# harmony-one/harmony

Measured on AMD Instinct MI355X. Metric: BLS12-381 aggregate-verifies/sec (committee=4096), higher is better.
Workload: dtype u64; 1 GPU; config2: committee=4096 masked aggregate + pairing verify, batch=262144/step, masks Bernoulli(0.9) seed 42, 48B staking commit payloads; parallelism=dp1 (per-shard replicas, no collective)

## Files before the change

### harmony_amd/core.py

```python
import ctypes
import os

_DIR = os.path.dirname(os.path.abspath(__file__))
_SO = os.environ.get("HBLS_SO", os.path.join(_DIR, "libhbls.so"))

HBLS_OK = 1
HBLS_FALSE = 0
HBLS_ERR = -1
HBLS_ERR_NOGPU = -2
HBLS_ERR_BADINPUT = -3
HBLS_NOQUORUM = -4
NOQUORUM = HBLS_NOQUORUM
TWO_THIRDS_DEC = 666666666666666667


class HblsError(RuntimeError):
    pass


class NoGpuError(HblsError):
    pass


class BadInputError(HblsError, ValueError):
# ... 68 lines not shown
    lib.hbls_vote_key_sums.argtypes = [
        ctypes.c_void_p, ctypes.POINTER(ctypes.c_uint32),
        ctypes.POINTER(ctypes.c_uint32), ctypes.c_size_t, ctypes.c_char_p,
        ctypes.POINTER(ctypes.c_int32)]
    lib.hbls_batch_verify_votes_multi.argtypes = [
        ctypes.c_void_p, ctypes.POINTER(ctypes.c_uint32),
        ctypes.POINTER(ctypes.c_uint32), ctypes.c_char_p, ctypes.c_char_p,
        ctypes.c_size_t, ctypes.c_size_t, ctypes.POINTER(ctypes.c_int32)]
    lib.hbls_stream_process_multi.argtypes = [
        ctypes.c_void_p, ctypes.POINTER(ctypes.c_uint32),
        ctypes.POINTER(ctypes.c_uint32), ctypes.POINTER(ctypes.c_uint32),
        ctypes.c_char_p, ctypes.POINTER(ctypes.c_uint32), ctypes.c_int,
        ctypes.c_size_t, ctypes.POINTER(ctypes.c_int32)]
    lib.hbls_rlc_last_stats.argtypes = [ctypes.POINTER(ctypes.c_uint32)]
    lib.hbls_rlc_last_stats.restype = None
    lib.hbls_set_agg_verify_mode.argtypes = [ctypes.c_int]
    lib.hbls_set_aggrlc_threshold.argtypes = [ctypes.c_int]
    lib.hbls_set_aggrlc_threshold.restype = None
    lib.hbls_aggrlc_last_stats.argtypes = [ctypes.POINTER(ctypes.c_uint32)]
    lib.hbls_aggrlc_last_stats.restype = None
    lib.hbls_set_aggrlc_final.argtypes = [ctypes.c_int]
    lib.hbls_aggrlc_final_selftest.argtypes = [ctypes.c_int]
    lib.hbls_set_aggrlc_sigleg.argtypes = [ctypes.c_int]
    lib.hbls_aggrlc_probe.argtypes = [ctypes.c_int, ctypes.c_char_p, ctypes.c_size_t,
                                      ctypes.c_char_p]
    lib.hbls_last_host_ns.restype = ctypes.c_uint64
    lib.hbls_last_host_ns.argtypes = [ctypes.c_int]
    u64p, u32p, i32p = (ctypes.POINTER(t) for t in
                        (ctypes.c_uint64, ctypes.c_uint32, ctypes.c_int32))
    lib.hbls_committee_set_quorum.argtypes = [ctypes.c_void_p, u64p, ctypes.c_uint64]
    lib.hbls_mask_power.argtypes = [ctypes.c_void_p, ctypes.c_char_p, ctypes.c_size_t,
                                    u64p, u32p]
    lib.hbls_agg_verify_quorum.argtypes = lib.hbls_agg_verify.argtypes
    lib.hbls_batch_agg_verify_quorum.argtypes = lib.hbls_batch_agg_verify.argtypes
    lib.hbls_batch_seal_verify_quorum.argtypes = lib.hbls_batch_seal_verify.argtypes
    lib.hbls_stream_power.argtypes = [ctypes.c_void_p, u32p, ctypes.c_int,
                                      u64p, u32p, i32p]
    lib.hbls_last_stage_ns.argtypes = [ctypes.c_int]
    lib.hbls_copy_bench_ns.restype = ctypes.c_uint64
    lib.hbls_copy_bench_ns.argtypes = [ctypes.c_size_t]
    lib.hbls_fpmul_bench_waves.restype = ctypes.c_double
    lib.hbls_fpmul_bench_waves.argtypes = [ctypes.c_int, ctypes.c_int]
    lib.hbls_coop_selftest.restype = ctypes.c_int
    lib.hbls_fpmul_asm_check.restype = ctypes.c_longlong
    lib.hbls_arith_probe.argtypes = [ctypes.c_int, ctypes.c_char_p, ctypes.c_size_t,
                                     ctypes.c_char_p, i32p]
# ... 76 lines not shown

def aggrlc_chunk_size() -> int:
    return _lib.hbls_aggrlc_chunk_size()


def aggrlc_last_stats():
    out = (ctypes.c_uint32 * 3)()
    _lib.hbls_aggrlc_last_stats(out)
    return list(out)


def set_aggrlc_final(kernel: int):
    _check(_lib.hbls_set_aggrlc_final(kernel), "set_aggrlc_final")


def aggrlc_final_selftest(nchunks: int) -> int:
    return _check(_lib.hbls_aggrlc_final_selftest(nchunks), "aggrlc_final_selftest")


def set_aggrlc_sigleg(leg: int):
    _check(_lib.hbls_set_aggrlc_sigleg(leg), "set_aggrlc_sigleg")


AGGRLC_PROBE_OPS = {"g1_mul64w": (0, 3 * 48 + 8, 3 * 48),
                    "g2_mul64w": (1, 6 * 48 + 8, 6 * 48),
                    "miller1_fe": (2, 6 * 48, 12 * 48)}


def aggrlc_probe(name: str, data: bytes, n_items: int) -> bytes:
    op, in_b, out_b = AGGRLC_PROBE_OPS[name]
    if len(data) != n_items * in_b:
        raise ValueError("aggrlc_probe: operand size")
    out = ctypes.create_string_buffer(max(1, n_items * out_b))
    _check(_lib.hbls_aggrlc_probe(op, data, n_items, out), "aggrlc_probe")
    return out.raw[:n_items * out_b]


def last_host_ns(i: int) -> int:
    return _lib.hbls_last_host_ns(i)


def pk_from_sk(sk32: bytes) -> bytes:
    out = ctypes.create_string_buffer(48)
    _check(_lib.hbls_pk_from_sk(sk32, out), "pk_from_sk")
    return out.raw

# ... 489 lines not shown
```

### harmony_amd/csrc/hbls_aggrlc.inc

```

#define AGGRLC_CHUNK 64
#define AGGRLC_WINDOWS 8


DEV void aggrlc_recode64(uint64_t k, uint64_t &mag, uint32_t &neg, uint32_t &top) {
    uint32_t c = 0;
    mag = 0; neg = 0;
#pragma unroll
    for (int j = 0; j < 16; j++) {
        uint32_t v = ((uint32_t)(k >> (4 * j)) & 15u) + c;
        uint32_t nx = j < 15 ? ((uint32_t)(k >> (4 * j + 4)) & 15u) : 0u;
        c = (v > 8u || (v == 8u && nx >= 8u)) ? 1u : 0u;
        uint32_t m = c ? 16u - v : v;
        mag |= (uint64_t)m << (4 * j);
        neg |= (c && m) ? (1u << j) : 0u;
    }
    top = c;
}

DEVN void g1_mul64w(g1_t &r, const g1_t &p, uint64_t k) {
    g1_t tab[8];
    tab[0] = p;
    g1_dbl(tab[1], tab[0]);
    g1_add(tab[2], tab[1], tab[0]);
// ... 104 lines not shown
    g1aff_t pa, ca;
    { fp_t t, ti, zi, zi2, zi3;
      fp_mul(t, A.z, C.z);
      fp_inv(ti, t);
      fp_mul(zi, ti, C.z);
      fp_sqr(zi2, zi);
      fp_mul(zi3, zi2, zi);
      fp_mul(pa.x, A.x, zi2);
      fp_mul(pa.y, A.y, zi3);
      fp_mul(zi, ti, A.z);
      fp_sqr(zi2, zi);
      fp_mul(zi3, zi2, zi);
      fp_mul(ca.x, C.x, zi2);
      fp_mul(ca.y, C.y, zi3); }
    g2aff_t ha;
    g2_t hmc = hms[i];
    g2_to_affine(ha, hmc);
    miller_loop2(f, ha, pa, sigs[i], ca);
    F[i] = f;
    elig[i] = 1;
    results[i] = 1;
}

__global__ void k_aggrlc_sigscale(const g1_t *aggpubs, const g2aff_t *sigs,
                                  const int32_t *sig_flags, const int32_t *hm_ok,
                                  const uint64_t *scalars, g2_t *B, int32_t *elig,
                                  int32_t *results, int batch) {
    int i = blockIdx.x * blockDim.x + threadIdx.x;
    if (i >= batch) return;
    g2_t b;
    g2_set_inf(b);
    elig[i] = 0;
    if (!hm_ok[i] || sig_flags[i] == 0) {
        results[i] = HBLS_ERR_BADINPUT; B[i] = b; return;
    }
    bool sig_inf = sig_flags[i] == 2;
    bool pub_inf = g1_is_inf(aggpubs[i]);
    if (pub_inf || sig_inf) {
        results[i] = (pub_inf && sig_inf) ? 1 : 0;
        B[i] = b; return;
    }
    uint64_t r = scalars[i];
    if (r == 0) r = 1;
    g2_t s;
    g2_from_affine(s, sigs[i]);
    g2_mul64w(b, s, r);
    B[i] = b;
    elig[i] = 1;
    results[i] = 1;
}

__global__ void __launch_bounds__(AGGRLC_CHUNK) k_aggrlc_sigsum(
        const g2_t *B, int batch, int nchunks, g2aff_t *S, int32_t *sflag) {
    int c = blockIdx.x;
    if (c >= nchunks) return;
    __shared__ g2_t red[AGGRLC_CHUNK];
    size_t i = (size_t)c * AGGRLC_CHUNK + threadIdx.x;
    if (i < (size_t)batch) red[threadIdx.x] = B[i];
    else g2_set_inf(red[threadIdx.x]);
    __syncthreads();
    for (int s = AGGRLC_CHUNK / 2; s > 0; s >>= 1) {
        if (threadIdx.x < s) {
            g2_t t;
            g2_add(t, red[threadIdx.x], red[threadIdx.x + s]);
            red[threadIdx.x] = t;
        }
        __syncthreads();
    }
    if (threadIdx.x == 0) {
        g2_t sum = red[0];
        if (g2_is_inf(sum)) {
            sflag[c] = 0;
        } else {
            g2aff_t a;
            g2_to_affine(a, sum);
            S[c] = a;
            sflag[c] = 1;
        }
    }
}

__global__ void k_aggrlc_miller1(const g1_t *aggpubs, const g2_t *hms,
                                 const uint64_t *scalars, const g2aff_t *S,
                                 const int32_t *sflag, fp12_t *F, int32_t *elig,
                                 int32_t *results, int batch, int nchunks) {
    size_t i = (size_t)blockIdx.x * blockDim.x + threadIdx.x;
    if (i >= (size_t)batch + (size_t)nchunks) return;
    fp12_t f;
    g2aff_t Q;
    g1aff_t P;
    bool run = false;
    if (i < (size_t)batch) {
        if (elig[i] == 1) {
            uint64_t r = scalars[i];
            if (r == 0) r = 1;
            g1_t A;
            g1_mul64w(A, aggpubs[i], r);
            if (g1_is_inf(A)) {
                elig[i] = 2; results[i] = 0;
            } else {
                g1_to_affine(P, A);
                g2_t hmc = hms[i];
                g2_to_affine(Q, hmc);
                run = true;
            }
        }
    } else {
        size_t c = i - (size_t)batch;
        if (sflag[c]) {
            Q = S[c];
            fp_load(P.x, BLS_G1_X);
            fp_t gy;
            fp_load(gy, BLS_G1_Y);
            fp_neg(P.y, gy);
            run = true;
        }
    }
    if (run) miller_loop1_h(f, Q, P);
    else fp12_one(f);
    F[i] = f;
}

__global__ void __launch_bounds__(AGGRLC_CHUNK) k_aggrlc_chunk_prod(
        const fp12_t *F, const int32_t *elig, int batch, int nchunks,
        fp12_t *FC, int32_t *ccnt, int32_t *cforce, const fp12_t *FX) {
    int c = blockIdx.x;
    if (c >= nchunks) return;
    __shared__ fp12_t red[AGGRLC_CHUNK];
    size_t i = (size_t)c * AGGRLC_CHUNK + threadIdx.x;
    int e = i < (size_t)batch ? elig[i] : 0;
    if (e == 1) red[threadIdx.x] = F[i];
    else fp12_one(red[threadIdx.x]);
    int cnt = __syncthreads_count(e != 0);
    int force = __syncthreads_or(e == 2);
    for (int s = AGGRLC_CHUNK / 2; s > 0; s >>= 1) {
        if (threadIdx.x < s) {
            fp12_t t;
            fp12_mul(t, red[threadIdx.x], red[threadIdx.x + s]);
            red[threadIdx.x] = t;
        }
        __syncthreads();
    }
    if (threadIdx.x == 0) {
// ... 111 lines not shown
    return g_aggrlc_final;
}
extern "C" int hbls_set_aggrlc_final(int kernel) {
    if (kernel == -1) kernel = AGGRLC_FINAL_DEFAULT;
    if (kernel != 0 && kernel != 8 && kernel != 16) return HBLS_ERR_BADINPUT;
    g_aggrlc_final = kernel;
    return HBLS_OK;
}
#define AGGRLC_SIGLEG_MIN_BATCH 16384
static int g_aggrlc_sigleg = -2;
static int aggrlc_sigleg(size_t batch) {
    if (g_aggrlc_sigleg == -2) {
        const char *e = getenv("HBLS_AGGRLC_SIGLEG");
        int k = e ? atoi(e) : -1;
        g_aggrlc_sigleg = (k == 0 || k == 1) ? k : -1;
    }
    if (g_aggrlc_sigleg >= 0) return g_aggrlc_sigleg;
    return batch >= AGGRLC_SIGLEG_MIN_BATCH ? 1 : 0;
}
extern "C" int hbls_set_aggrlc_sigleg(int leg) {
    if (leg < -1 || leg > 1) return HBLS_ERR_BADINPUT;
    g_aggrlc_sigleg = leg;
    return HBLS_OK;
}

static void launch_aggrlc_final(int kernel, const fp12_t *d_FC, const int32_t *d_ccnt,
                                const int32_t *d_cforce, int32_t *d_verdict, int nc) {
    if (kernel == 16)
        hipLaunchKernelGGL(k_aggrlc_final_coop<16>, dim3((uint32_t)((nc + 15) / 16)),
                           dim3(16 * CV_LANES), 0, 0, d_FC, d_ccnt, d_cforce, d_verdict, nc);
    else if (kernel == 8)
        hipLaunchKernelGGL(k_aggrlc_final_coop<8>, dim3((uint32_t)((nc + 7) / 8)),
                           dim3(8 * CV_LANES), 0, 0, d_FC, d_ccnt, d_cforce, d_verdict, nc);
    else
        hipLaunchKernelGGL(k_aggrlc_final, dim3((uint32_t)((nc + 63) / 64)), dim3(64), 0, 0,
                           d_FC, d_ccnt, d_cforce, d_verdict, nc);
}

__global__ void k_aggrlc_final_fill(fp12_t *FC, int32_t *ccnt, int32_t *cforce, int nchunks) {
    int c = blockIdx.x * blockDim.x + threadIdx.x;
    if (c >= nchunks) return;
    int kind = c % 8;
    fp_t one;
    fp_one(one);
    fp_t co[12];
    for (int k = 0; k < 12; k++) {
// ... 65 lines not shown
                       dp2.as<g1aff_t>(), 64, dwj.as<g1_t>(), AGGRLC_WINDOWS);
    hipLaunchKernelGGL(k_wtab_to_affine, dim3((int)((m + 255) / 256)), dim3(256), 0, 0,
                       dwj.as<g1_t>(), d_gt, dwi.as<uint8_t>(), m);
    std::vector<uint8_t> winf(m);
    bool ok = hipDeviceSynchronize() == hipSuccess &&
              hipMemcpy(winf.data(), dwi.p, m, hipMemcpyDeviceToHost) == hipSuccess;
    for (size_t k = 0; ok && k < m; k++)
        if (winf[k]) ok = false;
    if (!ok) { hipFree(d_gt); return HBLS_ERR; }
    g_aggrlc_gtab = d_gt;
    return HBLS_OK;
}

static bool aggrlc_wanted(size_t batch) {
    int m = agg_verify_mode();
    if (m == 0 || !g_aggrlc_gtab) return false;
    if (batch > RLC_MAX_ITEMS || (long long)batch < (long long)g_aggrlc_threshold) return false;
    if (m == 1) return true;
    return (int)batch > coop_threshold() && rf_mode() == 0 && !use_batch_affine();
}

static int aggrlc_verify(const g1_t *d_agg, const g2_t *d_hm, const g2aff_t *d_saff,
                         const int32_t *d_sflags, const int32_t *d_hok,
                         int32_t *d_res, size_t batch) {
    size_t nc = (batch + AGGRLC_CHUNK - 1) / AGGRLC_CHUNK;
    const int leg = aggrlc_sigleg(batch);
    const size_t nx = leg ? nc : 0;
    std::vector<uint64_t> scalars(batch);
    if (!rlc_draw_scalars(scalars.data(), batch)) return AGGRLC_FALLBACK;
    FreeClock fclk;
    uint64_t t_alloc = host_now_ns();
    const size_t f_bytes = (batch + nx) * sizeof(fp12_t);
    const size_t b_bytes = leg ? batch * sizeof(g2_t) : 0;
    DevBuf dsc(batch * 8), dF(f_bytes + b_bytes + nx * sizeof(g2aff_t)), delig(batch * 4);
    DevBuf dFC(nc * sizeof(fp12_t)), dcs((3 * nc + nx) * 4);
    g_host_ns[0] += host_now_ns() - t_alloc;
    FreeClockArm farm(fclk);
    if (dsc.err || dF.err || delig.err || dFC.err || dcs.err) {
        (void)hipGetLastError();
        return AGGRLC_FALLBACK;
    }
    fp12_t *d_F = dF.as<fp12_t>();
    g2_t *d_B = (g2_t *)((uint8_t *)dF.p + f_bytes);
    g2aff_t *d_S = (g2aff_t *)((uint8_t *)dF.p + f_bytes + b_bytes);
    EventSet<1> up;
    if (up.err != hipSuccess) return HBLS_ERR;
    HIP_OK(upload_then_wait(dsc.p, scalars.data(), batch * 8, up[0]));
    int32_t *d_ccnt = dcs.as<int32_t>(), *d_cforce = d_ccnt + nc, *d_verdict = d_cforce + nc;
    int32_t *d_sf = d_verdict + nc;
    EventSet<5> ev;
    if (ev.err != hipSuccess) return HBLS_ERR;
    (void)hipEventRecord(ev[0], 0);
    if (leg) {
        hipLaunchKernelGGL(k_aggrlc_sigscale, dim3((uint32_t)((batch + 63) / 64)), dim3(64), 0, 0,
                           d_agg, d_saff, d_sflags, d_hok, dsc.as<uint64_t>(), d_B,
                           delig.as<int32_t>(), d_res, (int)batch);
        hipLaunchKernelGGL(k_aggrlc_sigsum, dim3((uint32_t)nc), dim3(AGGRLC_CHUNK), 0, 0,
                           d_B, (int)batch, (int)nc, d_S, d_sf);
    }
    (void)hipEventRecord(ev[1], 0);
    if (leg)
        hipLaunchKernelGGL(k_aggrlc_miller1, dim3((uint32_t)((batch + nc + 63) / 64)), dim3(64),
                           0, 0, d_agg, d_hm, dsc.as<uint64_t>(), d_S, d_sf, d_F,
                           delig.as<int32_t>(), d_res, (int)batch, (int)nc);
    else
        hipLaunchKernelGGL(k_aggrlc_miller, dim3((uint32_t)((batch + 63) / 64)), dim3(64), 0, 0,
                           d_agg, d_hm, d_saff, d_sflags, d_hok, dsc.as<uint64_t>(),
                           g_aggrlc_gtab, d_F, delig.as<int32_t>(), d_res, (int)batch);
    (void)hipEventRecord(ev[2], 0);
    hipLaunchKernelGGL(k_aggrlc_chunk_prod, dim3((uint32_t)nc), dim3(AGGRLC_CHUNK), 0, 0,
                       d_F, delig.as<int32_t>(), (int)batch, (int)nc,
                       dFC.as<fp12_t>(), d_ccnt, d_cforce,
                       leg ? d_F + batch : (const fp12_t *)nullptr);
    (void)hipEventRecord(ev[3], 0);
    launch_aggrlc_final(aggrlc_final_kernel(), dFC.as<fp12_t>(), d_ccnt, d_cforce,
                        d_verdict, (int)nc);
    (void)hipEventRecord(ev[4], 0);
    std::vector<int32_t> hc(3 * nc);
    hipError_t e = hipMemcpy(hc.data(), dcs.p, 3 * nc * 4, hipMemcpyDeviceToHost);
    if (e == hipSuccess) e = hipGetLastError();
    for (int i = 0; i < 4; i++) {
        float ms = 0;
        if (e == hipSuccess && (i || leg)) (void)hipEventElapsedTime(&ms, ev[i], ev[i + 1]);
        g_stage_ns[i ? 3 + i : 7] = (uint64_t)(ms * 1e6);
    }
    HIP_OK(e);

    std::vector<uint32_t> failed;
    for (size_t c = 0; c < nc; c++) {
        if (hc[c] <= 0) continue;
        g_aggrlc_stats[0]++;
        if (hc[2 * nc + c] == 1) continue;
        g_aggrlc_stats[1]++;
        failed.push_back((uint32_t)c);
    }
    if (failed.empty()) return HBLS_OK;

    std::vector<int32_t> helig(batch);
    HIP_OK(hipMemcpy(helig.data(), delig.p, batch * 4, hipMemcpyDeviceToHost));
    std::vector<uint32_t> sel;
    for (uint32_t c : failed)
        for (size_t i = (size_t)c * AGGRLC_CHUNK;
             i < batch && i < ((size_t)c + 1) * AGGRLC_CHUNK; i++)
            if (helig[i]) sel.push_back((uint32_t)i);
    size_t ns = sel.size();
    g_aggrlc_stats[2] = (uint32_t)ns;
    if (!ns) return HBLS_OK;
    DevBuf dsel(ns * 4);
    if (dsel.err) return HBLS_ERR;
    HIP_OK(hipMemcpy(dsel.p, sel.data(), ns * 4, hipMemcpyHostToDevice));
    hipLaunchKernelGGL(k_verify_sel, dim3((uint32_t)((ns + 63) / 64)), dim3(64), 0, 0,
                       dsel.as<uint32_t>(), (int)ns, d_agg, d_hm, d_saff, d_sflags, d_hok,
                       d_res, (int)batch);
    HIP_OK(hipGetLastError());
    return HBLS_OK;
}

enum { AGGRLC_PROBE_G1_MUL64W = 0, AGGRLC_PROBE_G2_MUL64W = 1, AGGRLC_PROBE_MILLER1_FE = 2,
       AGGRLC_PROBE_N_OPS = 3 };
#define AGGRLC_PROBE_MAX_ITEMS 4096
__global__ void k_aggrlc_probe(int op, const uint64_t *in, int in_w, uint64_t *out, int out_w,
                               int n) {
// ... 44 lines not shown
```

### harmony_amd/csrc/hbls_ctxset.inc

```

#define CX_VALID 1u
#define CX_PREP_T 160
#define CX_MSG_SLOT 48

struct cx_ctx {
    const g1aff_t *table;
    const g1_t *full_sum;
    const g1aff_t *wtab;
    const uint8_t *winf;
    const uint64_t *power;
    uint64_t threshold;
    uint32_t n;
    uint32_t uniform;
    uint32_t q_set;
    uint32_t pad;
};

struct cx_item {
    uint32_t ctx;
    uint32_t bm_off;
    uint32_t flags;
    uint32_t pad;
};

// ... 343 lines not shown
        hipLaunchKernelGGL(k_ctx_prepare, dim3(cx_blocks(batch * CX_PREP_T)), dim3(256), 0, 0,
                           s->d_ctx, (uint32_t)s->n_ctx, dci.as<uint32_t>(),
                           dblob.as<uint8_t>(), dboff.as<uint32_t>(), 96u, dmsgs.as<uint8_t>(),
                           dmoff.as<uint32_t>(), batch, ditems.as<cx_item>(), dst.as<int32_t>(),
                           dsig.as<uint8_t>(), dmsg.as<uint8_t>());
        if (quorum)
            hipLaunchKernelGGL(k_ctx_mask_power, dim3(cx_blocks(batch * 64)),
                               dim3(CX_MP_THREADS), 0, 0, s->d_ctx, ditems.as<cx_item>(),
                               dblob.as<uint8_t>(), (int)batch, 1, (uint64_t *)nullptr,
                               (uint32_t *)nullptr, dst.as<int32_t>());
        tm.stop_and_store();
        front_ns = g_last_ns;
    }
    HIP_OK(hipGetLastError());
    g_stage_ns[7] = front_ns;
    std::vector<int32_t> status(batch);
    HIP_OK(hipMemcpy(status.data(), dst.p, batch * 4, hipMemcpyDeviceToHost));
    std::vector<uint32_t> idx;
    for (size_t j = 0; j < batch; j++)
        if (status[j] == HBLS_OK) idx.push_back((uint32_t)j);
    size_t nlive = idx.size();
    aggrlc_stats_reset();
    for (int i = 0; i < 7; i++) g_stage_ns[i] = 0;
    if (nlive == 0) {
        for (size_t j = 0; j < batch; j++) results[j] = status[j];
        return HBLS_OK;
    }

    DevBuf didx(nlive * 4), gitems(nlive * sizeof(cx_item)), gsig(nlive * 96),
           gmsg(nlive * CX_MSG_SLOT);
    DevBuf dagg(nlive * sizeof(g1_t)), dhm(nlive * sizeof(g2_t));
    DevBuf dsaff(nlive * sizeof(g2aff_t)), dsflags(nlive * 4), dhok(nlive * 4), dres(nlive * 4);
    if (didx.err || gitems.err || gsig.err || gmsg.err || dagg.err || dhm.err || dsaff.err ||
        dsflags.err || dhok.err || dres.err) return HBLS_ERR;
    EventSet<8> ev;
    if (ev.err != hipSuccess) return HBLS_ERR;
    uint64_t t_launch = host_now_ns();
    const cx_item *l_items = ditems.as<cx_item>();
    const uint8_t *l_sig = dsig.as<uint8_t>(), *l_msg = dmsg.as<uint8_t>();
    (void)hipEventRecord(ev[2], 0);
    if (nlive < batch) {
        HIP_OK(hipMemcpy(didx.p, idx.data(), nlive * 4, hipMemcpyHostToDevice));
        hipLaunchKernelGGL(k_ctx_gather, dim3(cx_blocks(nlive * CX_PREP_T)), dim3(256), 0, 0,
                           didx.as<uint32_t>(), nlive, l_items, l_sig, l_msg,
                           gitems.as<cx_item>(), gsig.as<uint8_t>(), gmsg.as<uint8_t>());
        l_items = gitems.as<cx_item>();
// ... 39 lines not shown
```

### harmony_amd/csrc/hbls_dev.hip

```cpp
#include <hip/hip_runtime.h>
#include <stdint.h>
#include <string.h>
#include <stdio.h>
#include <stdlib.h>
#include "../../oracle/bls_consts.h"
#include "../../include/hbls.h"

typedef unsigned __int128 u128;

#define DEV __device__ __forceinline__
#define DEVN __device__ __noinline__

struct fp_t { uint64_t l[6]; };
struct fp2_t { fp_t a, b; };

DEV bool fp_is_zero(const fp_t &x) {
    return (x.l[0] | x.l[1] | x.l[2] | x.l[3] | x.l[4] | x.l[5]) == 0;
}
DEV bool fp_eq(const fp_t &x, const fp_t &y) {
    uint64_t d = 0;
#pragma unroll
    for (int i = 0; i < 6; i++) d |= x.l[i] ^ y.l[i];
    return d == 0;
}
// ... 2079 lines not shown
__global__ void k_keccak(const uint8_t *msgs, int mlen, uint8_t *outs, int batch) {
    int i = blockIdx.x * blockDim.x + threadIdx.x;
    if (i >= batch) return;
    keccak256_dev(msgs + (size_t)i * mlen, mlen, outs + (size_t)i * 32);
}

#include "hbls_coop.inc"

#include <mutex>
#include <vector>

static int g_device = -1;
static int g_fast_cofactor = 1;
static int g_coop_threshold = -1;
static int coop_threshold(void) {
    if (g_coop_threshold < 0) {
        const char *e = getenv("HBLS_COOP_THRESHOLD");
        g_coop_threshold = e ? atoi(e) : 8192;
    }
    return g_coop_threshold;
}
extern "C" void hbls_set_coop_threshold(int n) { g_coop_threshold = n; }
static thread_local uint64_t g_last_ns = 0;
static thread_local uint64_t g_stage_ns[8] = {0};
static std::once_flag g_init_flag;
static int g_init_rc = HBLS_ERR_NOGPU;
static int aggrlc_init_tables(void);
static bool aggrlc_wanted(size_t batch);
static void aggrlc_stats_reset(void);

#define HIP_OK(expr) do { hipError_t _e = (expr); if (_e != hipSuccess) { \
    fprintf(stderr, "hbls: %s failed: %s\n", #expr, hipGetErrorString(_e)); return HBLS_ERR; } } while (0)
#define HIP_OKP(expr) do { hipError_t _e = (expr); if (_e != hipSuccess) { \
    fprintf(stderr, "hbls: %s failed: %s\n", #expr, hipGetErrorString(_e)); return nullptr; } } while (0)

extern "C" int hbls_device_count(void) {
    int n = 0;
    if (hipGetDeviceCount(&n) != hipSuccess) return 0;
    return n;
}

extern "C" int hbls_init(int device) {
    int n = hbls_device_count();
    if (n <= 0) return HBLS_ERR_NOGPU;
    if (device >= 0) {
        if (device >= n) return HBLS_ERR_BADINPUT;
        if (hipSetDevice(device) != hipSuccess) return HBLS_ERR;
        g_device = device;
    } else {
        hipGetDevice(&g_device);
    }
    void *p = nullptr;
    if (hipMalloc(&p, 64) != hipSuccess) return HBLS_ERR;
    hipFree(p);
    g_init_rc = HBLS_OK;
    (void)aggrlc_init_tables();
    return HBLS_OK;
}

extern "C" void hbls_set_g2_cofactor_mode(int fast) { g_fast_cofactor = fast; }
extern "C" const char *hbls_version(void) { return "hbls 0.1 (gfx950)"; }
extern "C" uint64_t hbls_last_kernel_ns(void) { return g_last_ns; }
extern "C" uint64_t hbls_last_stage_ns(int i) { return (i >= 0 && i < 8) ? g_stage_ns[i] : 0; }

static int require_gpu(void) {
    if (g_init_rc != HBLS_OK) {
        if (hbls_init(-1) != HBLS_OK) return HBLS_ERR_NOGPU;
    }
    return HBLS_OK;
}

struct DevBuf {
    void *p = nullptr;
    hipError_t err = hipSuccess;
    explicit DevBuf(size_t n) { err = hipMalloc(&p, n ? n : 1); }
    ~DevBuf() { if (p) hipFree(p); }
    template <typename T> T *as() const { return (T *)p; }
};

#include <chrono>
static thread_local uint64_t g_host_ns[5] = {0};
static thread_local bool g_host_open = false;
static inline uint64_t host_now_ns(void) {
    return (uint64_t)std::chrono::duration_cast<std::chrono::nanoseconds>(
        std::chrono::steady_clock::now().time_since_epoch()).count();
}
// ... 320 lines not shown
}
extern "C" size_t hbls_committee_size(const hbls_committee_t *c) { return c->n; }

extern "C" int hbls_mask_aggregate_g1(const hbls_committee_t *c, const uint8_t *bitmap,
                                      uint8_t out48[48]) {
    int rc = require_gpu();
    if (rc != HBLS_OK) return rc;
    size_t bm = (c->n + 7) / 8;
    DevBuf dbm(bm), dout(sizeof(g1_t)), dser(48);
    if (dbm.err || dout.err || dser.err) return HBLS_ERR;
    HIP_OK(hipMemcpy(dbm.p, bitmap, bm, hipMemcpyHostToDevice));
    Timer tm;
    launch_mask_aggregate(c->d_table, (int)c->n, dbm.as<uint8_t>(), (int)bm,
                          c->d_full_sum, dout.as<g1_t>(), 1,
                          c->d_wtab, c->d_winf);
    hipLaunchKernelGGL(k_g1_serialize, dim3(1), dim3(1), 0, 0,
                       dout.as<g1_t>(), dser.as<uint8_t>(), 1);
    tm.stop_and_store();
    HIP_OK(hipGetLastError());
    HIP_OK(hipMemcpy(out48, dser.p, 48, hipMemcpyDeviceToHost));
    return HBLS_OK;
}

static int aggrlc_verify(const g1_t *d_agg, const g2_t *d_hm, const g2aff_t *d_saff,
                         const int32_t *d_sflags, const int32_t *d_hok,
                         int32_t *d_res, size_t batch);
#define AGGRLC_FALLBACK 2

struct AggHostSrc { const uint8_t *bitmaps, *sigs, *msgs; };

static int run_agg_verify_pairing(const g1_t *d_agg, g2_t *d_hm, g2aff_t *d_saff,
                                  int32_t *d_sflags, int32_t *d_hok, int32_t *d_res,
                                  size_t batch, size_t mode_batch, const EventSet<8> &ev,
                                  uint64_t t_launch, int32_t *results) {
    int nb = (int)((batch + 63) / 64);
    (void)hipEventRecord(ev[6], 0);
    int arc = AGGRLC_FALLBACK;
    if (aggrlc_wanted(mode_batch)) {
        arc = aggrlc_verify(d_agg, d_hm, d_saff, d_sflags, d_hok, d_res, batch);
        if (arc != HBLS_OK && arc != AGGRLC_FALLBACK) return arc;
    }
    if (arc == HBLS_OK) {
    } else if ((int)batch <= coop_threshold()) {
        LAUNCH_COOP(k_verify_coop, batch, d_agg, d_hm, d_saff, d_sflags, d_hok, d_res,
                    (int)batch);
    } else if (rf_mode() == 0 && use_batch_affine()) {
        DevBuf dpa(batch * sizeof(g1aff_t)), dpi(batch * 4), dha(batch * sizeof(g2aff_t));
        if (dpa.err || dpi.err || dha.err) return HBLS_ERR;
        int nba = (int)((batch + 64 * BA_K - 1) / (64 * BA_K));
        hipLaunchKernelGGL(k_g1_batch_affine, dim3(nba), dim3(64), 0, 0,
                           d_agg, dpa.as<g1aff_t>(), dpi.as<int32_t>(), (int)batch);
        hipLaunchKernelGGL(k_g2_batch_affine, dim3(nba), dim3(64), 0, 0,
                           d_hm, dha.as<g2aff_t>(), d_hok, (int)batch);
        hipLaunchKernelGGL(k_verify_aff, dim3(nb), dim3(64), 0, 0,
                           dpa.as<g1aff_t>(), dpi.as<int32_t>(), dha.as<g2aff_t>(),
                           d_saff, d_sflags, d_hok, d_res, (int)batch);
        HIP_OK(hipDeviceSynchronize());
    } else {
        LAUNCH_VERIFY_SCALAR(nb, d_agg, d_hm, d_saff, d_sflags, d_hok, d_res, (int)batch);
    }
    (void)hipEventRecord(ev[7], 0);
    HIP_OK(hipEventSynchronize(ev[7]));
    float ms_total = 0, ms = 0;
    (void)hipEventElapsedTime(&ms_total, ev[2], ev[7]);
    g_last_ns = (uint64_t)(ms_total * 1e6);
    for (int i = 0; i < 4; i++) {
        (void)hipEventElapsedTime(&ms, ev[2 * i], ev[2 * i + 1]);
        g_stage_ns[i] = (uint64_t)(ms * 1e6);
    }
    HIP_OK(hipGetLastError());
    HIP_OK(hipMemcpy(results, d_res, batch * 4, hipMemcpyDeviceToHost));
    g_host_ns[2] += host_now_ns() - t_launch;
    return HBLS_OK;
}

static int run_agg_verify_pipeline(const hbls_committee_t *c, const uint8_t *d_bm,
                                   const uint8_t *d_sig, const uint8_t *d_msg,
                                   size_t msg_len, size_t batch, int32_t *results,
                                   const AggHostSrc *src = nullptr) {
    HostCall hcall;
    size_t bm = (c->n + 7) / 8;
    FreeClock fclk;
    uint64_t t_alloc = host_now_ns();
    DevBuf dagg(batch * sizeof(g1_t)), dhm(batch * sizeof(g2_t));
    DevBuf dsaff(batch * sizeof(g2aff_t)), dsflags(batch * 4), dhok(batch * 4), dres(batch * 4);
    g_host_ns[0] += host_now_ns() - t_alloc;
    FreeClockArm farm(fclk);
    if (dagg.err || dhm.err || dsaff.err || dsflags.err || dhok.err || dres.err)
        return HBLS_ERR;
    int nb = (int)((batch + 63) / 64);
    aggrlc_stats_reset();
    for (int i = 4; i < 8; i++) g_stage_ns[i] = 0;
    EventSet<8> ev;
    EventSet<3> up;
    if (ev.err != hipSuccess || up.err != hipSuccess) return HBLS_ERR;
    uint64_t t_launch = host_now_ns();

    if (src) HIP_OK(upload_then_wait((void *)d_msg, src->msgs, batch * msg_len, up[0]));
    (void)hipEventRecord(ev[2], 0);
    if ((int)batch <= coop_threshold()) {
        int nbc = (int)((batch + CV_ITEMS - 1) / CV_ITEMS);
        LAUNCH_COOP(k_hash_to_g2_coop, batch, d_msg, (int)msg_len, dhm.as<g2_t>(), dhok.as<int32_t>(),
                           (int)batch, g_fast_cofactor);
    } else {
        hipLaunchKernelGGL(k_hash_to_g2, dim3(nb), dim3(64), 0, 0,
                           d_msg, (int)msg_len, dhm.as<g2_t>(), dhok.as<int32_t>(),
                           (int)batch, g_fast_cofactor);
    }
    (void)hipEventRecord(ev[3], 0);

    if (src) HIP_OK(upload_then_wait((void *)d_sig, src->sigs, batch * 96, up[1]));
    (void)hipEventRecord(ev[4], 0);
    if ((int)batch <= coop_threshold()) {
        int nbc = (int)((batch + CV_ITEMS - 1) / CV_ITEMS);
        LAUNCH_COOP(k_g2_decompress_coop, batch, d_sig, dsaff.as<g2aff_t>(), dsflags.as<int32_t>(), (int)batch);
    } else {
        hipLaunchKernelGGL(k_g2_decompress, dim3(nb), dim3(64), 0, 0,
                           d_sig, dsaff.as<g2aff_t>(), dsflags.as<int32_t>(), (int)batch);
    }
    (void)hipEventRecord(ev[5], 0);

    if (src) HIP_OK(upload_then_wait((void *)d_bm, src->bitmaps, batch * bm, up[2]));
    (void)hipEventRecord(ev[0], 0);
    launch_mask_aggregate(c->d_table, (int)c->n, d_bm, (int)bm,
                                         c->d_full_sum, dagg.as<g1_t>(), (int)batch,
                                         c->d_wtab, c->d_winf);
    (void)hipEventRecord(ev[1], 0);

    return run_agg_verify_pairing(dagg.as<g1_t>(), dhm.as<g2_t>(), dsaff.as<g2aff_t>(),
                                  dsflags.as<int32_t>(), dhok.as<int32_t>(), dres.as<int32_t>(),
                                  batch, batch, ev, t_launch, results);
}

extern "C" int hbls_batch_agg_verify(const hbls_committee_t *c, const uint8_t *bitmaps,
                                     const uint8_t *sigs96, const uint8_t *msgs,
                                     size_t msg_len, size_t batch, int32_t *results) {
    int rc = require_gpu();
    if (rc != HBLS_OK) return rc;
    HostCall hcall;
    size_t bm = (c->n + 7) / 8;
    FreeClock fclk;
    uint64_t t_alloc = host_now_ns();
    DevBuf dbm(batch * bm), dsig(batch * 96), dmsg(batch * msg_len);
    g_host_ns[0] += host_now_ns() - t_alloc;
    FreeClockArm farm(fclk);
    if (dbm.err || dsig.err || dmsg.err) return HBLS_ERR;
    AggHostSrc src = { bitmaps, sigs96, msgs };
    return run_agg_verify_pipeline(c, dbm.as<uint8_t>(), dsig.as<uint8_t>(),
                                   dmsg.as<uint8_t>(), msg_len, batch, results, &src);
}

extern "C" int hbls_agg_verify(const hbls_committee_t *c, const uint8_t *bitmap,
                               const uint8_t sig96[96], const uint8_t *msg, size_t msg_len) {
    int32_t r;
// ... 1529 lines not shown
```

### include/hbls.h

```cpp
#ifndef HBLS_H
#define HBLS_H

#include <stddef.h>
#include <stdint.h>

#ifdef __cplusplus
extern "C" {
#endif

enum {
    HBLS_OK = 1,
    HBLS_FALSE = 0,
    HBLS_ERR = -1,
    HBLS_ERR_NOGPU = -2,
    HBLS_ERR_BADINPUT = -3,
    HBLS_NOQUORUM = -4,
};

#define HBLS_TWO_THIRDS_DEC 666666666666666667ULL

int hbls_init(int device);

int hbls_device_count(void);

// ... 132 lines not shown


int hbls_vote_key_sums(const hbls_committee_t *c, const uint32_t *key_off,
                       const uint32_t *key_idx, size_t batch,
                       uint8_t *out48s, int32_t *ok);

int hbls_batch_verify_votes_multi(const hbls_committee_t *c, const uint32_t *key_off,
                                  const uint32_t *key_idx, const uint8_t *sigs96,
                                  const uint8_t *msgs, size_t msg_len, size_t batch,
                                  int32_t *results);

int hbls_stream_process_multi(hbls_stream_t *s, const uint32_t *key_off,
                              const uint32_t *key_idx, const uint32_t *round_idx,
                              const uint8_t *sigs96, const uint32_t *active_slots,
                              int n_active, size_t batch, int32_t *results);

int hbls_set_agg_verify_mode(int mode);
void hbls_set_aggrlc_threshold(int min_batch);
int hbls_aggrlc_chunk_size(void);
void hbls_aggrlc_last_stats(uint32_t out[3]);
int hbls_set_aggrlc_final(int kernel);
int hbls_aggrlc_final_selftest(int nchunks);
int hbls_set_aggrlc_sigleg(int leg);

int hbls_batch_keccak256(const uint8_t *msgs, size_t msg_len, size_t batch,
                         uint8_t *out32s);

const char *hbls_version(void);
double hbls_mad_peak_ops(void);
uint64_t hbls_last_kernel_ns(void);
uint64_t hbls_last_host_ns(int i);

#ifdef __cplusplus
}
#endif
#endif
```

Measured before the change: 776,800 aggregate-verifies/sec.

## Start signature-scaling leg early and overlap chunk Miller loops on a side stream

Adds an early path for large batches: before the bitmap upload and mask aggregation, it launches the random-scalar signature scaling and per-chunk signature sums. It also launches the per-chunk Miller loops against the generator on a high-priority side stream using a cooperative LDS kernel. The check for an infinite aggregated pubkey is deferred into the miller1 kernel, which marks affected chunks dirty and recomputes only those chunk sums and Miller legs afterwards. The aim is to hide the signature leg behind the pubkey aggregation work. The cost is extra streams, events, buffers and a repair pass.

```diff
diff --git a/harmony_amd/core.py b/harmony_amd/core.py
--- a/harmony_amd/core.py
+++ b/harmony_amd/core.py
@@ -114,6 +114,8 @@
     lib.hbls_set_aggrlc_final.argtypes = [ctypes.c_int]
     lib.hbls_aggrlc_final_selftest.argtypes = [ctypes.c_int]
     lib.hbls_set_aggrlc_sigleg.argtypes = [ctypes.c_int]
+    lib.hbls_set_aggrlc_early.argtypes = [ctypes.c_int]
+    lib.hbls_set_aggrlc_chunkleg.argtypes = [ctypes.c_int]
     lib.hbls_aggrlc_probe.argtypes = [ctypes.c_int, ctypes.c_char_p, ctypes.c_size_t,
                                       ctypes.c_char_p]
     lib.hbls_last_host_ns.restype = ctypes.c_uint64
@@ -236,6 +238,14 @@
     _check(_lib.hbls_set_aggrlc_sigleg(leg), "set_aggrlc_sigleg")
 
 
+def set_aggrlc_early(early: int):
+    _check(_lib.hbls_set_aggrlc_early(early), "set_aggrlc_early")
+
+
+def set_aggrlc_chunkleg(kernel: int):
+    _check(_lib.hbls_set_aggrlc_chunkleg(kernel), "set_aggrlc_chunkleg")
+
+
 AGGRLC_PROBE_OPS = {"g1_mul64w": (0, 3 * 48 + 8, 3 * 48),
                     "g2_mul64w": (1, 6 * 48 + 8, 6 * 48),
                     "miller1_fe": (2, 6 * 48, 12 * 48)}
diff --git a/harmony_amd/csrc/hbls_aggrlc.inc b/harmony_amd/csrc/hbls_aggrlc.inc
--- a/harmony_amd/csrc/hbls_aggrlc.inc
+++ b/harmony_amd/csrc/hbls_aggrlc.inc
@@ -150,6 +150,9 @@
     results[i] = 1;
 }
 
+#define AGGRLC_ELIG_OPEN 3
+
+template <bool HOISTED>
 __global__ void k_aggrlc_sigscale(const g1_t *aggpubs, const g2aff_t *sigs,
                                   const int32_t *sig_flags, const int32_t *hm_ok,
                                   const uint64_t *scalars, g2_t *B, int32_t *elig,
@@ -163,10 +166,14 @@
         results[i] = HBLS_ERR_BADINPUT; B[i] = b; return;
     }
     bool sig_inf = sig_flags[i] == 2;
-    bool pub_inf = g1_is_inf(aggpubs[i]);
-    if (pub_inf || sig_inf) {
-        results[i] = (pub_inf && sig_inf) ? 1 : 0;
-        B[i] = b; return;
+    if (HOISTED) {
+        if (sig_inf) { elig[i] = AGGRLC_ELIG_OPEN; B[i] = b; return; }
+    } else {
+        bool pub_inf = g1_is_inf(aggpubs[i]);
+        if (pub_inf || sig_inf) {
+            results[i] = (pub_inf && sig_inf) ? 1 : 0;
+            B[i] = b; return;
+        }
     }
     uint64_t r = scalars[i];
     if (r == 0) r = 1;
@@ -178,13 +185,16 @@
     results[i] = 1;
 }
 
+template <bool REPAIR>
 __global__ void __launch_bounds__(AGGRLC_CHUNK) k_aggrlc_sigsum(
-        const g2_t *B, int batch, int nchunks, g2aff_t *S, int32_t *sflag) {
+        const g2_t *B, int batch, int nchunks, g2aff_t *S, int32_t *sflag,
+        const int32_t *elig, const int32_t *dirty) {
     int c = blockIdx.x;
     if (c >= nchunks) return;
+    if (REPAIR && !dirty[c]) return;
     __shared__ g2_t red[AGGRLC_CHUNK];
     size_t i = (size_t)c * AGGRLC_CHUNK + threadIdx.x;
-    if (i < (size_t)batch) red[threadIdx.x] = B[i];
+    if (i < (size_t)batch && (!REPAIR || elig[i] != 0)) red[threadIdx.x] = B[i];
     else g2_set_inf(red[threadIdx.x]);
     __syncthreads();
     for (int s = AGGRLC_CHUNK / 2; s > 0; s >>= 1) {
@@ -208,10 +218,12 @@
     }
 }
 
+template <bool HOISTED>
 __global__ void k_aggrlc_miller1(const g1_t *aggpubs, const g2_t *hms,
                                  const uint64_t *scalars, const g2aff_t *S,
                                  const int32_t *sflag, fp12_t *F, int32_t *elig,
-                                 int32_t *results, int batch, int nchunks) {
+                                 int32_t *results, int batch, int nchunks,
+                                 int32_t *dirty) {
     size_t i = (size_t)blockIdx.x * blockDim.x + threadIdx.x;
     if (i >= (size_t)batch + (size_t)nchunks) return;
     fp12_t f;
@@ -219,6 +231,17 @@
     g1aff_t P;
     bool run = false;
     if (i < (size_t)batch) {
+        if (HOISTED) {
+            int32_t e = elig[i];
+            if (e == AGGRLC_ELIG_OPEN) {
+                results[i] = g1_is_inf(aggpubs[i]) ? 1 : 0;
+                elig[i] = 0;
+            } else if (e == 1 && g1_is_inf(aggpubs[i])) {
+                results[i] = 0;
+                elig[i] = 0;
+                dirty[i / AGGRLC_CHUNK] = 1;
+            }
+        }
         if (elig[i] == 1) {
             uint64_t r = scalars[i];
             if (r == 0) r = 1;
@@ -247,6 +270,91 @@
     if (run) miller_loop1_h(f, Q, P);
     else fp12_one(f);
     F[i] = f;
+}
+
+__global__ void k_aggrlc_chunkleg(const g2aff_t *S, const int32_t *sflag,
+                                  const int32_t *dirty, fp12_t *FX, int nchunks) {
+    int c = blockIdx.x * blockDim.x + threadIdx.x;
+    if (c >= nchunks) return;
+    if (dirty && !dirty[c]) return;
+    fp12_t f;
+    if (sflag[c]) {
+        g2aff_t Q = S[c];
+        g1aff_t P;
+        fp_load(P.x, BLS_G1_X);
+        fp_t gy;
+        fp_load(gy, BLS_G1_Y);
+        fp_neg(P.y, gy);
+        miller_loop1_h(f, Q, P);
+    } else {
+        fp12_one(f);
+    }
+    FX[c] = f;
+}
+
+DEVN void cv_miller1(lds_fp2 *A, int q) {
+    if (q == 0) {
+        lds_st(A + CV_T1, lds_ld(A + CV_Q1));
+        lds_st(A + (CV_T1 + 1), lds_ld(A + (CV_Q1 + 1)));
+        fp2_t one; fp_one(one.a); fp_zero(one.b);
+        lds_st(A + (CV_T1 + 2), one);
+    }
+    __syncthreads();
+    cv_fp12_set_one(A, q, CV_F0);
+    int cur = CV_F0, oth = CV_F1;
+    for (int bit = 62; bit >= 0; bit--) {
+        cv_fp12_sqr(A, q, oth, cur);
+        { int s = cur; cur = oth; oth = s; }
+        cv_ml_dbl_step(A, q, CV_T1, CV_PP);
+        cv_fp12_mul_line(A, q, oth, cur);
+        { int s = cur; cur = oth; oth = s; }
+        if ((BLS_U >> bit) & 1) {
+            cv_ml_add_step(A, q, CV_T1, CV_Q1, CV_PP);
+            cv_fp12_mul_line(A, q, oth, cur);
+            { int s = cur; cur = oth; oth = s; }
+        }
+    }
+    if (cur != CV_F0) cv_fp12_copy(A, q, CV_F0, cur);
+}
+
+template <int ITEMS>
+__global__ void __launch_bounds__(ITEMS * CV_LANES) k_aggrlc_chunkleg_coop(
+        const g2aff_t *S, const int32_t *sflag, fp12_t *FX, int nchunks) {
+    __shared__ uint64_t arena[ITEMS][CV_STRIDE64];
+    __shared__ int32_t pre[ITEMS];
+    const int sub = threadIdx.x / CV_LANES;
+    const int q = threadIdx.x % CV_LANES;
+    const int c = blockIdx.x * ITEMS + sub;
+    lds_fp2 *A = (lds_fp2 *)arena[sub];
+    if (q == 0) {
+        int32_t r = -1;
+        if (c < nchunks) r = sflag[c] ? 1 : 0;
+        pre[sub] = r;
+        g2aff_t Q;
+        if (r == 1) {
+            Q = S[c];
+        } else {
+            fp_load(Q.x.a, BLS_G2_XA); fp_load(Q.x.b, BLS_G2_XB);
+            fp_load(Q.y.a, BLS_G2_YA); fp_load(Q.y.b, BLS_G2_YB);
+        }
+        lds_st(A + (CV_Q1), Q.x); lds_st(A + (CV_Q1 + 1), Q.y);
+        fp2_t p;
+        fp_t gy;
+        fp_load(p.a, BLS_G1_X); fp_load(gy, BLS_G1_Y);
+        fp_neg(p.b, gy);
+        lds_st(A + (CV_PP), p);
+    }
+    __syncthreads();
+    cv_miller1(A, q);
+    if (q == 0) {
+        int32_t r = pre[sub];
+        if (r != -1) {
+            fp12_t f;
+            if (r == 1) cv_ld_fp12(A, CV_F0, f);
+            else fp12_one(f);
+            FX[c] = f;
+        }
+    }
 }
 
 __global__ void __launch_bounds__(AGGRLC_CHUNK) k_aggrlc_chunk_prod(
@@ -404,6 +512,127 @@
     if (leg < -1 || leg > 1) return HBLS_ERR_BADINPUT;
     g_aggrlc_sigleg = leg;
     return HBLS_OK;
+}
+
+#define AGGRLC_EARLY_MIN_BATCH 262144
+static int g_aggrlc_early = -2;
+static int aggrlc_early(size_t batch) {
+    if (g_aggrlc_early == -2) {
+        const char *e = getenv("HBLS_AGGRLC_EARLY");
+        int k = e ? atoi(e) : -1;
+        g_aggrlc_early = (k == 0 || k == 1) ? k : -1;
+    }
+    if (g_aggrlc_early >= 0) return g_aggrlc_early;
+    return batch >= AGGRLC_EARLY_MIN_BATCH ? 1 : 0;
+}
+extern "C" int hbls_set_aggrlc_early(int early) {
+    if (early < -1 || early > 1) return HBLS_ERR_BADINPUT;
+    g_aggrlc_early = early;
+    return HBLS_OK;
+}
+
+#define AGGRLC_CHUNKLEG_DEFAULT 16
+static int g_aggrlc_chunkleg = -2;
+static int aggrlc_chunkleg_kernel(void) {
+    if (g_aggrlc_chunkleg == -2) {
+        const char *e = getenv("HBLS_AGGRLC_CHUNKLEG");
+        int k = e ? atoi(e) : AGGRLC_CHUNKLEG_DEFAULT;
+        g_aggrlc_chunkleg = (k == 0 || k == 16) ? k : AGGRLC_CHUNKLEG_DEFAULT;
+    }
+    return g_aggrlc_chunkleg;
+}
+extern "C" int hbls_set_aggrlc_chunkleg(int kernel) {
+    if (kernel == -1) kernel = AGGRLC_CHUNKLEG_DEFAULT;
+    if (kernel != 0 && kernel != 16) return HBLS_ERR_BADINPUT;
+    g_aggrlc_chunkleg = kernel;
+    return HBLS_OK;
+}
+
+static hipStream_t g_aggrlc_side_stream = nullptr;
+static std::once_flag g_aggrlc_side_flag;
+static hipStream_t aggrlc_side_stream(void) {
+    std::call_once(g_aggrlc_side_flag, [] {
+        hipStream_t s = nullptr;
+        int least = 0, greatest = 0;
+        if (hipDeviceGetStreamPriorityRange(&least, &greatest) != hipSuccess) {
+            (void)hipGetLastError();
+            greatest = 0;
+        }
+        if (hipStreamCreateWithPriority(&s, hipStreamNonBlocking, greatest) == hipSuccess)
+            g_aggrlc_side_stream = s;
+        else
+            (void)hipGetLastError();
+    });
+    return g_aggrlc_side_stream;
+}
+
+struct AggrlcEarly {
+    size_t batch, nc;
+    std::vector<uint64_t> scalars;
+    DevBuf dsc, dB, dS, dFX, delig, dflag;
+    EventSet<5> ev;
+    bool launched = false;
+    AggrlcEarly(size_t b, size_t n)
+        : batch(b), nc(n), scalars(b), dsc(b * 8), dB(b * sizeof(g2_t)),
+          dS(n * sizeof(g2aff_t)), dFX(n * sizeof(fp12_t)), delig(b * 4), dflag(2 * n * 4) {}
+    bool ok() const {
+        return !dsc.err && !dB.err && !dS.err && !dFX.err && !delig.err && !dflag.err &&
+               ev.err == hipSuccess;
+    }
+    int32_t *sflag() const { return dflag.as<int32_t>(); }
+    int32_t *dirty() const { return dflag.as<int32_t>() + nc; }
+    ~AggrlcEarly() {
+        HostSpan sp(3);
+        if (launched) (void)hipStreamSynchronize(g_aggrlc_side_stream);
+    }
+};
+static void aggrlc_early_free(AggrlcEarly *e) { delete e; }
+
+static AggrlcEarly *aggrlc_early_begin(const g2aff_t *d_saff, const int32_t *d_sflags,
+                                       const int32_t *d_hok, int32_t *d_res, size_t batch) {
+    if (!aggrlc_wanted(batch) || !aggrlc_sigleg(batch) || !aggrlc_early(batch)) return nullptr;
+    hipStream_t side = aggrlc_side_stream();
+    if (!side) return nullptr;
+    size_t nc = (batch + AGGRLC_CHUNK - 1) / AGGRLC_CHUNK;
+    uint64_t t_alloc = host_now_ns();
+    AggrlcEarly *st = new (std::nothrow) AggrlcEarly(batch, nc);
+    g_host_ns[0] += host_now_ns() - t_alloc;
+    if (!st) return nullptr;
+    if (!st->ok() || !rlc_draw_scalars(st->scalars.data(), batch)) {
+        (void)hipGetLastError();
+        delete st;
+        return nullptr;
+    }
+    bool good = upload_then_wait(st->dsc.p, st->scalars.data(), batch * 8, st->ev[4]) == hipSuccess;
+    st->launched = true;
+    good = good && hipMemsetAsync(st->dirty(), 0, nc * 4, 0) == hipSuccess;
+    if (!good) {
+        (void)hipGetLastError();
+        (void)hipDeviceSynchronize();
+        delete st;
+        return nullptr;
+    }
+    (void)hipEventRecord(st->ev[0], 0);
+    hipLaunchKernelGGL(k_aggrlc_sigscale<true>, dim3((uint32_t)((batch + 63) / 64)), dim3(64), 0, 0,
+                       (const g1_t *)nullptr, d_saff, d_sflags, d_hok, st->dsc.as<uint64_t>(),
+                       st->dB.as<g2_t>(), st->delig.as<int32_t>(), d_res, (int)batch);
+    hipLaunchKernelGGL(k_aggrlc_sigsum<false>, dim3((uint32_t)nc), dim3(AGGRLC_CHUNK), 0, 0,
+                       st->dB.as<g2_t>(), (int)batch, (int)nc, st->dS.as<g2aff_t>(), st->sflag(),
+                       (const int32_t *)nullptr, (const int32_t *)nullptr);
+    (void)hipEventRecord(st->ev[1], 0);
+    (void)hipStreamWaitEvent(side, st->ev[1], 0);
+    (void)hipEventRecord(st->ev[2], side);
+    (void)hipStreamWaitEvent(0, st->ev[2], 0);
+    if (aggrlc_chunkleg_kernel() == 16)
+        hipLaunchKernelGGL(k_aggrlc_chunkleg_coop<16>, dim3((uint32_t)((nc + 15) / 16)),
+                           dim3(16 * CV_LANES), 0, side, st->dS.as<g2aff_t>(), st->sflag(),
+                           st->dFX.as<fp12_t>(), (int)nc);
+    else
+        hipLaunchKernelGGL(k_aggrlc_chunkleg, dim3((uint32_t)((nc + 63) / 64)), dim3(64), 0, side,
+                           st->dS.as<g2aff_t>(), st->sflag(), (const int32_t *)nullptr,
+                           st->dFX.as<fp12_t>(), (int)nc);
+    (void)hipEventRecord(st->ev[3], side);
+    return st;
 }
 
 static void launch_aggrlc_final(int kernel, const fp12_t *d_FC, const int32_t *d_ccnt,
@@ -515,17 +744,18 @@
 
 static int aggrlc_verify(const g1_t *d_agg, const g2_t *d_hm, const g2aff_t *d_saff,
                          const int32_t *d_sflags, const int32_t *d_hok,
-                         int32_t *d_res, size_t batch) {
+                         int32_t *d_res, size_t batch, AggrlcEarly *early) {
     size_t nc = (batch + AGGRLC_CHUNK - 1) / AGGRLC_CHUNK;
-    const int leg = aggrlc_sigleg(batch);
-    const size_t nx = leg ? nc : 0;
-    std::vector<uint64_t> scalars(batch);
-    if (!rlc_draw_scalars(scalars.data(), batch)) return AGGRLC_FALLBACK;
+    const int leg = early ? 1 : aggrlc_sigleg(batch);
+    const size_t nx = (leg && !early) ? nc : 0;
+    std::vector<uint64_t> scalars(early ? 0 : batch);
+    if (!early && !rlc_draw_scalars(scalars.data(), batch)) return AGGRLC_FALLBACK;
     FreeClock fclk;
     uint64_t t_alloc = host_now_ns();
     const size_t f_bytes = (batch + nx) * sizeof(fp12_t);
-    const size_t b_bytes = leg ? batch * sizeof(g2_t) : 0;
-    DevBuf dsc(batch * 8), dF(f_bytes + b_bytes + nx * sizeof(g2aff_t)), delig(batch * 4);
+    const size_t b_bytes = nx ? batch * sizeof(g2_t) : 0;
+    DevBuf dsc(early ? 0 : batch * 8), dF(f_bytes + b_bytes + nx * sizeof(g2aff_t));
+    DevBuf delig(early ? 0 : batch * 4);
     DevBuf dFC(nc * sizeof(fp12_t)), dcs((3 * nc + nx) * 4);
     g_host_ns[0] += host_now_ns() - t_alloc;
     FreeClockArm farm(fclk);
@@ -536,35 +766,51 @@
     fp12_t *d_F = dF.as<fp12_t>();
     g2_t *d_B = (g2_t *)((uint8_t *)dF.p + f_bytes);
     g2aff_t *d_S = (g2aff_t *)((uint8_t *)dF.p + f_bytes + b_bytes);
+    const uint64_t *d_sc = early ? early->dsc.as<uint64_t>() : dsc.as<uint64_t>();
+    int32_t *d_elig = early ? early->delig.as<int32_t>() : delig.as<int32_t>();
     EventSet<1> up;
     if (up.err != hipSuccess) return HBLS_ERR;
-    HIP_OK(upload_then_wait(dsc.p, scalars.data(), batch * 8, up[0]));
+    if (!early) HIP_OK(upload_then_wait(dsc.p, scalars.data(), batch * 8, up[0]));
     int32_t *d_ccnt = dcs.as<int32_t>(), *d_cforce = d_ccnt + nc, *d_verdict = d_cforce + nc;
     int32_t *d_sf = d_verdict + nc;
     EventSet<5> ev;
     if (ev.err != hipSuccess) return HBLS_ERR;
     (void)hipEventRecord(ev[0], 0);
-    if (leg) {
-        hipLaunchKernelGGL(k_aggrlc_sigscale, dim3((uint32_t)((batch + 63) / 64)), dim3(64), 0, 0,
-                           d_agg, d_saff, d_sflags, d_hok, dsc.as<uint64_t>(), d_B,
-                           delig.as<int32_t>(), d_res, (int)batch);
-        hipLaunchKernelGGL(k_aggrlc_sigsum, dim3((uint32_t)nc), dim3(AGGRLC_CHUNK), 0, 0,
-                           d_B, (int)batch, (int)nc, d_S, d_sf);
+    if (leg && !early) {
+        hipLaunchKernelGGL(k_aggrlc_sigscale<false>, dim3((uint32_t)((batch + 63) / 64)), dim3(64),
+                           0, 0, d_agg, d_saff, d_sflags, d_hok, d_sc, d_B,
+                           d_elig, d_res, (int)batch);
+        hipLaunchKernelGGL(k_aggrlc_sigsum<false>, dim3((uint32_t)nc), dim3(AGGRLC_CHUNK), 0, 0,
+                           d_B, (int)batch, (int)nc, d_S, d_sf,
+                           (const int32_t *)nullptr, (const int32_t *)nullptr);
     }
     (void)hipEventRecord(ev[1], 0);
-    if (leg)
-        hipLaunchKernelGGL(k_aggrlc_miller1, dim3((uint32_t)((batch + nc + 63) / 64)), dim3(64),
-                           0, 0, d_agg, d_hm, dsc.as<uint64_t>(), d_S, d_sf, d_F,
-                           delig.as<int32_t>(), d_res, (int)batch, (int)nc);
-    else
+    if (early) {
+        hipLaunchKernelGGL(k_aggrlc_miller1<true>, dim3((uint32_t)((batch + 63) / 64)), dim3(64),
+                           0, 0, d_agg, d_hm, d_sc, early->dS.as<g2aff_t>(), early->sflag(), d_F,
+                           d_elig, d_res, (int)batch, 0, early->dirty());
+        (void)hipStreamWaitEvent(0, early->ev[3], 0);
+        hipLaunchKernelGGL(k_aggrlc_sigsum<true>, dim3((uint32_t)nc), dim3(AGGRLC_CHUNK), 0, 0,
+                           early->dB.as<g2_t>(), (int)batch, (int)nc, early->dS.as<g2aff_t>(),
+                           early->sflag(), d_elig, early->dirty());
+        hipLaunchKernelGGL(k_aggrlc_chunkleg, dim3((uint32_t)((nc + 63) / 64)), dim3(64), 0, 0,
+                           early->dS.as<g2aff_t>(), early->sflag(), early->dirty(),
+                           early->dFX.as<fp12_t>(), (int)nc);
+    } else if (leg) {
+        hipLaunchKernelGGL(k_aggrlc_miller1<false>, dim3((uint32_t)((batch + nc + 63) / 64)),
+                           dim3(64), 0, 0, d_agg, d_hm, d_sc, d_S, d_sf, d_F,
+                           d_elig, d_res, (int)batch, (int)nc, (int32_t *)nullptr);
+    } else {
         hipLaunchKernelGGL(k_aggrlc_miller, dim3((uint32_t)((batch + 63) / 64)), dim3(64), 0, 0,
-                           d_agg, d_hm, d_saff, d_sflags, d_hok, dsc.as<uint64_t>(),
-                           g_aggrlc_gtab, d_F, delig.as<int32_t>(), d_res, (int)batch);
+                           d_agg, d_hm, d_saff, d_sflags, d_hok, d_sc,
+                           g_aggrlc_gtab, d_F, d_elig, d_res, (int)batch);
+    }
     (void)hipEventRecord(ev[2], 0);
     hipLaunchKernelGGL(k_aggrlc_chunk_prod, dim3((uint32_t)nc), dim3(AGGRLC_CHUNK), 0, 0,
-                       d_F, delig.as<int32_t>(), (int)batch, (int)nc,
+                       d_F, d_elig, (int)batch, (int)nc,
                        dFC.as<fp12_t>(), d_ccnt, d_cforce,
-                       leg ? d_F + batch : (const fp12_t *)nullptr);
+                       early ? early->dFX.as<fp12_t>()
+                             : leg ? d_F + batch : (const fp12_t *)nullptr);
     (void)hipEventRecord(ev[3], 0);
     launch_aggrlc_final(aggrlc_final_kernel(), dFC.as<fp12_t>(), d_ccnt, d_cforce,
                         d_verdict, (int)nc);
@@ -574,8 +820,17 @@
     if (e == hipSuccess) e = hipGetLastError();
     for (int i = 0; i < 4; i++) {
         float ms = 0;
-        if (e == hipSuccess && (i || leg)) (void)hipEventElapsedTime(&ms, ev[i], ev[i + 1]);
+        if (e == hipSuccess && (i || (leg && !early)))
+            (void)hipEventElapsedTime(&ms, ev[i], ev[i + 1]);
         g_stage_ns[i ? 3 + i : 7] = (uint64_t)(ms * 1e6);
+    }
+    if (early && e == hipSuccess) {
+        float ms = 0;
+        (void)hipEventElapsedTime(&ms, early->ev[0], early->ev[1]);
+        g_stage_ns[7] = (uint64_t)(ms * 1e6);
+        ms = 0;
+        (void)hipEventElapsedTime(&ms, early->ev[2], early->ev[3]);
+        g_stage_ns[8] = (uint64_t)(ms * 1e6);
     }
     HIP_OK(e);
 
@@ -590,7 +845,7 @@
     if (failed.empty()) return HBLS_OK;
 
     std::vector<int32_t> helig(batch);
-    HIP_OK(hipMemcpy(helig.data(), delig.p, batch * 4, hipMemcpyDeviceToHost));
+    HIP_OK(hipMemcpy(helig.data(), d_elig, batch * 4, hipMemcpyDeviceToHost));
     std::vector<uint32_t> sel;
     for (uint32_t c : failed)
         for (size_t i = (size_t)c * AGGRLC_CHUNK;
diff --git a/harmony_amd/csrc/hbls_ctxset.inc b/harmony_amd/csrc/hbls_ctxset.inc
--- a/harmony_amd/csrc/hbls_ctxset.inc
+++ b/harmony_amd/csrc/hbls_ctxset.inc
@@ -389,6 +389,7 @@
     size_t nlive = idx.size();
     aggrlc_stats_reset();
     for (int i = 0; i < 7; i++) g_stage_ns[i] = 0;
+    g_stage_ns[8] = 0;
     if (nlive == 0) {
         for (size_t j = 0; j < batch; j++) results[j] = status[j];
         return HBLS_OK;
diff --git a/harmony_amd/csrc/hbls_dev.hip b/harmony_amd/csrc/hbls_dev.hip
--- a/harmony_amd/csrc/hbls_dev.hip
+++ b/harmony_amd/csrc/hbls_dev.hip
@@ -2125,7 +2125,7 @@
 }
 extern "C" void hbls_set_coop_threshold(int n) { g_coop_threshold = n; }
 static thread_local uint64_t g_last_ns = 0;
-static thread_local uint64_t g_stage_ns[8] = {0};
+static thread_local uint64_t g_stage_ns[9] = {0};
 static std::once_flag g_init_flag;
 static int g_init_rc = HBLS_ERR_NOGPU;
 static int aggrlc_init_tables(void);
@@ -2164,7 +2164,7 @@
 extern "C" void hbls_set_g2_cofactor_mode(int fast) { g_fast_cofactor = fast; }
 extern "C" const char *hbls_version(void) { return "hbls 0.1 (gfx950)"; }
 extern "C" uint64_t hbls_last_kernel_ns(void) { return g_last_ns; }
-extern "C" uint64_t hbls_last_stage_ns(int i) { return (i >= 0 && i < 8) ? g_stage_ns[i] : 0; }
+extern "C" uint64_t hbls_last_stage_ns(int i) { return (i >= 0 && i < 9) ? g_stage_ns[i] : 0; }
 
 static int require_gpu(void) {
     if (g_init_rc != HBLS_OK) {
@@ -2531,9 +2531,17 @@
     return HBLS_OK;
 }
 
+struct AggrlcEarly;
+static AggrlcEarly *aggrlc_early_begin(const g2aff_t *d_saff, const int32_t *d_sflags,
+                                       const int32_t *d_hok, int32_t *d_res, size_t batch);
+static void aggrlc_early_free(AggrlcEarly *e);
+struct AggrlcEarlyHold {
+    AggrlcEarly *p = nullptr;
+    ~AggrlcEarlyHold() { if (p) aggrlc_early_free(p); }
+};
 static int aggrlc_verify(const g1_t *d_agg, const g2_t *d_hm, const g2aff_t *d_saff,
                          const int32_t *d_sflags, const int32_t *d_hok,
-                         int32_t *d_res, size_t batch);
+                         int32_t *d_res, size_t batch, AggrlcEarly *early);
 #define AGGRLC_FALLBACK 2
 
 struct AggHostSrc { const uint8_t *bitmaps, *sigs, *msgs; };
@@ -2541,12 +2549,13 @@
 static int run_agg_verify_pairing(const g1_t *d_agg, g2_t *d_hm, g2aff_t *d_saff,
                                   int32_t *d_sflags, int32_t *d_hok, int32_t *d_res,
                                   size_t batch, size_t mode_batch, const EventSet<8> &ev,
-                                  uint64_t t_launch, int32_t *results) {
+                                  uint64_t t_launch, int32_t *results,
+                                  AggrlcEarly *early = nullptr) {
     int nb = (int)((batch + 63) / 64);
     (void)hipEventRecord(ev[6], 0);
     int arc = AGGRLC_FALLBACK;
-    if (aggrlc_wanted(mode_batch)) {
-        arc = aggrlc_verify(d_agg, d_hm, d_saff, d_sflags, d_hok, d_res, batch);
+    if (early || aggrlc_wanted(mode_batch)) {
+        arc = aggrlc_verify(d_agg, d_hm, d_saff, d_sflags, d_hok, d_res, batch, early);
         if (arc != HBLS_OK && arc != AGGRLC_FALLBACK) return arc;
     }
     if (arc == HBLS_OK) {
@@ -2577,6 +2586,7 @@
         (void)hipEventElapsedTime(&ms, ev[2 * i], ev[2 * i + 1]);
         g_stage_ns[i] = (uint64_t)(ms * 1e6);
     }
+    if (early && arc == HBLS_OK) g_stage_ns[3] += g_stage_ns[7];
     HIP_OK(hipGetLastError());
     HIP_OK(hipMemcpy(results, d_res, batch * 4, hipMemcpyDeviceToHost));
     g_host_ns[2] += host_now_ns() - t_launch;
@@ -2599,7 +2609,7 @@
         return HBLS_ERR;
     int nb = (int)((batch + 63) / 64);
     aggrlc_stats_reset();
-    for (int i = 4; i < 8; i++) g_stage_ns[i] = 0;
+    for (int i = 4; i < 9; i++) g_stage_ns[i] = 0;
     EventSet<8> ev;
     EventSet<3> up;
     if (ev.err != hipSuccess || up.err != hipSuccess) return HBLS_ERR;
@@ -2629,6 +2639,10 @@
     }
     (void)hipEventRecord(ev[5], 0);
 
+    AggrlcEarlyHold early;
+    early.p = aggrlc_early_begin(dsaff.as<g2aff_t>(), dsflags.as<int32_t>(), dhok.as<int32_t>(),
+                                 dres.as<int32_t>(), batch);
+
     if (src) HIP_OK(upload_then_wait((void *)d_bm, src->bitmaps, batch * bm, up[2]));
     (void)hipEventRecord(ev[0], 0);
     launch_mask_aggregate(c->d_table, (int)c->n, d_bm, (int)bm,
@@ -2638,7 +2652,7 @@
 
     return run_agg_verify_pairing(dagg.as<g1_t>(), dhm.as<g2_t>(), dsaff.as<g2aff_t>(),
                                   dsflags.as<int32_t>(), dhok.as<int32_t>(), dres.as<int32_t>(),
-                                  batch, batch, ev, t_launch, results);
+                                  batch, batch, ev, t_launch, results, early.p);
 }
 
 extern "C" int hbls_batch_agg_verify(const hbls_committee_t *c, const uint8_t *bitmaps,
diff --git a/include/hbls.h b/include/hbls.h
--- a/include/hbls.h
+++ b/include/hbls.h
@@ -178,6 +178,8 @@
 int hbls_set_aggrlc_final(int kernel);
 int hbls_aggrlc_final_selftest(int nchunks);
 int hbls_set_aggrlc_sigleg(int leg);
+int hbls_set_aggrlc_early(int early);
+int hbls_set_aggrlc_chunkleg(int kernel);
 
 int hbls_batch_keccak256(const uint8_t *msgs, size_t msg_len, size_t batch,
                          uint8_t *out32s);
```

New measurement: 814,900 aggregate-verifies/sec (median of 6 runs). 1.05x the previous value.
